# UniBwTAS/continuous_clustering

Measured on AMD Instinct MI355X. Metric: Mpoints/s clustered (64-beam streams), higher is better.
Workload: dtype f32

## Files before the change

continuous_clustering_amd/csrc/cc_k_assoc_global.h:

```cpp
#pragma once

constexpr int LINK_SLOTS_V1 = 8;

struct AssocCtx
{
    SP p;
    int R, NC, RC;
    float az_width, maxd2;
    int max_steps_in_row, max_steps_in_column, stop_enabled, stop_min_steps;
};

__device__ __forceinline__ int uf_find(int32_t* uf, int a)
{
    while (true)
    {
        const int pa = ld_agent(&uf[a]);
        if (pa == a)
            return a;
        const int gp = ld_agent(&uf[pa]);
        if (gp != pa)
            __hip_atomic_store(&uf[a], gp, __ATOMIC_RELAXED, __HIP_MEMORY_SCOPE_AGENT);
        a = pa;
    }
}
// ... 325 lines not shown
                    err = CC_ERR_CAPACITY;
                    err_a = n_unf + cnt;
                    break;
                }
                if (row < R)
                    p.root[lc * R + row] = active[k] ? rootc[k] : -1;
                if (is_new)
                {
                    const int cell = lc * R + row;
                    const int pos = n_unf + __popcll(mask & lanes_below());
                    const double fin = pcaz[k] + (double) mad[k];
                    tree_init(p, cell, fin);
                    p.ulist[pos] = cell;
                    p.t_pos[cell] = pos;
                    L = fin < L ? fin : L;
                }
                if (cnt > 0 && n_unf == 0)
                    M = gc;
                n_unf += cnt;
            }
            L = wave_min_f64(L);
            assoc_wave_sync();
#pragma unroll
            for (int k = 0; k < RPL; k++)
            {
                if (active[k] && parent[k] >= 0)
                {
                    const int r = rootc[k];
                    const long long rg = p.colg[r / R];
                    p.t_width[r] = (uint32_t) (gc - rg + 1);
                    const double cand = pcaz[k] + (double) mad[k];
                    atomicMax((unsigned long long*) &p.t_fin[r], (unsigned long long) __double_as_longlong(cand));
                    atomicAdd(&p.t_pts[r], 1u);
                }
            }
            assoc_wave_sync();
#pragma unroll
            for (int k = 0; k < RPL; k++)
            {
                const int row = k * 64 + lane;
                if (active[k] && parent[k] >= 0)
                {
                    const int rp = rootc[k];
                    for (int j = 0; j < nlinks[k]; j++)
                    {
                        const int rq = p.root[s_links[row][j]];
                        if (rq != rp && rq >= 0 && !p.t_finished[rp] && !p.t_finished[rq])
                        {
                            log_link(g, st, p.link_log, rp, rq);
                            uf_union(p.t_uf, rp, rq);
                        }
                    }
                }
            }
            assoc_wave_sync();
        }
        else
        {
            serial_cols++;
            if (lane == 0)
            {
                int nn = n_unf;
                double LL = L;
                long long MM = M;
                int e = 0;
                for (int row = 0; row < R; row++)
                {
                    const int ci = lc * R + row;
                    if (p.ignored[ci])
                    {
                        p.root[ci] = -1;
                        p.sc_parent[ci] = -2;
                        if (g.mirror_fields)
                            p.sc_visits[ci] = 0;
                        continue;
                    }
                    const float m = ccm::asinf_exact(cfg.max_distance / p.dist[ci]);
                    const double caz = cell_caz(cb, p.incaz[ci]);
                    int proot = -1, par = -1, nl = 0, vis = 0;
                    bool ov = false;
                    scan_point<true>(c, lc, gc, row, first_local, m, caz, proot, par, nullptr, nl, ov, LINK_SLOTS_V1, &vis, st, &g);
                    p.sc_parent[ci] = (int16_t) par;
                    if (g.mirror_fields)
                        p.sc_visits[ci] = sat_u16(vis);
                    if (proot == -1)
                    {
                        if (nn + 1 > g.tree_capacity)
                        {
                            e = CC_ERR_CAPACITY;
                            break;
                        }
                        proot = ci;
                        const double fin = caz + (double) m;
                        tree_init(p, ci, fin);
                        p.ulist[nn] = ci;
                        p.t_pos[ci] = nn;
                        if (nn == 0)
                            MM = gc;
                        nn++;
                        LL = fin < LL ? fin : LL;
                    }
                    p.root[ci] = proot;
                }
                s_bcast[0] = nn;
                s_bcast[1] = e;
                s_bd[0] = LL;
                s_bl[0] = MM;
            }
            assoc_wave_sync();
            n_unf = s_bcast[0];
            if (s_bcast[1])
            {
                err = s_bcast[1];
                err_a = n_unf;
            }
            L = s_bd[0];
            M = s_bl[0];
            assoc_wave_sync();
        }
        if (err)
            break;

        if (gc % nth != 0)
            continue;
        const double min_az = p.colminaz[lc];
        long long M_c;
        if (n_unf == 0)
            M_c = gc + 1;
        else if (min_az == last_min_az)
        {
            alias_rounds++;
            M_c = M;
        }
        else if (!(min_az >= L) && !((gc + 1 - M) >= NC))
            M_c = M;
        else
        {
            for (int i = lane; i < n_unf; i += 64)
            {
                p.agg_fin[i] = 0ull;
                p.agg_min[i] = 0x7fffffffffffffffll;
                p.agg_max[i] = 0;
                p.agg_pts[i] = 0;
                p.agg_first[i] = 0x7fffffff;
                p.agg_cid[i] = 0;
                p.agg_flag[i] = 0;
            }
            assoc_wave_sync();
            for (int i = lane; i < n_unf; i += 64)
            {
                const int t = p.ulist[i];
                const int rep = uf_find(p.t_uf, t);
                const int j = p.t_pos[rep];
                p.ucomp[i] = j;
                const long long tg = p.colg[t / R];
                atomicMax(&p.agg_fin[j], (unsigned long long) __double_as_longlong(ld_agent(&p.t_fin[t])));
                atomicMin(&p.agg_min[j], tg);
                atomicMax(&p.agg_max[j], tg + (long long) p.t_width[t]);
                atomicAdd(&p.agg_pts[j], ld_agent(&p.t_pts[t]));
                atomicMin(&p.agg_first[j], i);
            }
            assoc_wave_sync();
            int exceed_local = 0;
            for (int i = lane; i < n_unf; i += 64)
            {
                if (p.ucomp[i] == i)
                {
                    const double fin = __longlong_as_double((long long) ld_agent(&p.agg_fin[i]));
                    const bool unfinished = fin > min_az;
                    const bool exceeds = (ld_agent(&p.agg_max[i]) - ld_agent(&p.agg_min[i])) >= NC;
                    if (exceeds)
                        exceed_local++;
                    p.agg_flag[i] = (!unfinished || exceeds) ? 1 : 0;
                }
            }
            for (int o = 32; o > 0; o >>= 1)
                exceed_local += __shfl_xor(exceed_local, o);
            exceed += exceed_local;
            assoc_wave_sync();
            int last_first = -1;
            while (true)
            {
                int best = 0x7fffffff;
                for (int i = lane; i < n_unf; i += 64)
                    if (p.ucomp[i] == i && p.agg_flag[i] && ld_agent(&p.agg_pts[i]) > 5u)
                    {
                        const int fi = ld_agent(&p.agg_first[i]);
                        if (fi > last_first && fi < best)
                            best = fi;
                    }
                best = wave_min_i32(best);
                if (best == 0x7fffffff)
                    break;
                const int j = p.ucomp[best];
                const unsigned cid = (unsigned) cluster_counter;
                if (lane == 0)
                    p.agg_cid[j] = cid;
                emit(CC_EV_CLUSTER, ld_agent(&p.agg_min[j]), ld_agent(&p.agg_max[j]) - 1, cid, ld_agent(&p.agg_pts[j]), gc);
                cluster_counter++;
                clusters_finished++;
                last_first = best;
            }
            assoc_wave_sync();
            long long min_all = 0x7fffffffffffffffll, min_surv = 0x7fffffffffffffffll;
            double L_new = 1.7976931348623157e308;
            int out = 0;
            for (int base = 0; base < n_unf; base += 64)
            {
                const int i = base + lane;
                bool surv = false;
                int t = -1;
                if (i < n_unf)
                {
                    t = p.ulist[i];
                    const int j = p.ucomp[i];
                    const long long tg = p.colg[t / R];
                    min_all = tg < min_all ? tg : min_all;
                    if (p.agg_flag[j])
                    {
                        p.t_finished[t] = 1;
                        p.t_cid[t] = p.agg_cid[j];
                    }
                    else
                    {
                        surv = true;
                        min_surv = tg < min_surv ? tg : min_surv;
                        if (j == i)
                        {
                            const double fin = __longlong_as_double((long long) ld_agent(&p.agg_fin[i]));
                            L_new = fin < L_new ? fin : L_new;
                        }
                    }
                }
                const unsigned long long mask = __ballot(surv);
                if (surv)
                {
                    const int np = out + __popcll(mask & lanes_below());
                    p.ulist[np] = t;
                    p.t_pos[t] = np;
                }
                out += __popcll(mask);
            }
            min_all = wave_min_i64(min_all);
            min_surv = wave_min_i64(min_surv);
            L = wave_min_f64(L_new);
            M_c = min_all;
            M = min_surv;
            n_unf = out;
            assoc_wave_sync();
        }
        last_min_az = min_az;

        if (M_c < first_unpub)
        {
            err = CC_ERR_BOOKKEEPING;
            err_a = M_c;
            err_b = first_unpub;
            break;
        }
        const long long old_unpub = first_unpub, old_ring = ring_start;
        first_unpub = M_c;
        ring_start = first_unpub - NC > 0 ? first_unpub - NC : 0;
        emit(CC_EV_PUBLISH_COLUMNS, old_unpub, first_unpub - 1, 0, 0, gc);
        cells_published += (unsigned long long) (first_unpub - old_unpub) * (unsigned long long) R;
        (void) old_ring;
    }

    if (lane == 0)
    {
        st->first_unpublished = first_unpub;
        st->batch[slot].pub_end = first_unpub;
        st->ring_start = ring_start;
        st->cluster_counter = cluster_counter;
        st->n_unfinished = n_unf;
        st->min_required = M;
        st->finish_lower_bound = L;
        st->last_round_min_az = last_min_az;
        st->cells_published = cells_published;
        st->clusters_finished = clusters_finished;
        st->exceed_one_rotation = exceed;
        st->serial_columns = serial_cols;
        st->stamp_alias_rounds = alias_rounds;
        st->batch[slot].acp_next = col_end;
        if (err == 0)
            st->assoc_mode = (cfg.max_steps_in_row > WIN_COLS - 2 || n_unf * 2 > g.lds_tree_limit) ? 1 : 0;
        st->n_events = n_events < g.event_capacity ? n_events : g.event_capacity;
        if (g.record_events && n_events > g.event_capacity && err == 0)
        {
            err = CC_ERR_CAPACITY;
            err_a = n_events;
        }
        if (err)
            raise_error(st, err, err_a, err_b);
    }
}

template<int RPL>
__global__ __launch_bounds__(64) void k_associate(Geometry g, cc_config cfg, Planes P, StreamState* states, int first_stream, int slot)
{
    associate_stream<RPL>(g, cfg, P, states, first_stream + (int) blockIdx.x, slot);
}


template<int RPL, bool MIRROR>
__device__ __forceinline__ void scan_column_epilogue(const SP& p, const int R, const int lc, const int lane, const int (&parent)[RPL],
                                                     const int (&nlinks)[RPL], const double (&fin)[RPL], const unsigned long long (&packed)[RPL],
                                                     int reach)
{
    int t[RPL];
#pragma unroll
    for (int k = 0; k < RPL; k++)
    {
        const int row = k * 64 + lane;
        const bool same_col = parent[k] >= 0 && (parent[k] >> 8) == 0;
        t[k] = same_col ? (parent[k] & 0xff) : row;
    }
    for (int it = 0; it < 7; it++)
    {
        int nt[RPL];
        bool changed = false;
#pragma unroll
        for (int k = 0; k < RPL; k++)
        {
            const int src = t[k];
            const int lo = __shfl(t[0], src & 63);
            const int hi = RPL > 1 ? __shfl(t[RPL - 1], src & 63) : lo;
            nt[k] = src < 64 ? lo : hi;
            changed |= nt[k] != t[k];
        }
#pragma unroll
        for (int k = 0; k < RPL; k++)
            t[k] = nt[k];
        if (!__any(changed))
            break;
    }
    int cnt_new = 0, mine[RPL];
    int max_delta = 0;
    int flags = 0;
    int n_act = 0;
    double newfin = 1.7976931348623157e308;
#pragma unroll
    for (int k = 0; k < RPL; k++)
    {
        n_act |= __popcll(__ballot(parent[k] >= -1)) << (8 * k);
        const bool is_new = parent[k] == -1;
        const unsigned long long mask = __ballot(is_new);
        const int newidx = cnt_new + __popcll(mask & lanes_below());
        cnt_new += __popcll(mask);
        mine[k] = is_new ? newidx : (parent[k] >= 0 ? parent[k] : -1);
        if (is_new && fin[k] < newfin)
            newfin = fin[k];
        if (parent[k] >= 0)
        {
            int d = parent[k] >> 8;
            const int nl = nlinks[k] == 255 ? LINK_SLOTS : nlinks[k];
            for (int j = 0; j < nl; j++)
            {
                const int dj = (int) ((packed[k] >> (16 * j + 8)) & 0xff);
                d = dj > d ? dj : d;
            }
            max_delta = d > max_delta ? d : max_delta;
        }
        if (nlinks[k] == 255)
            flags |= 1;
        else if (nlinks[k] > 0)
            flags |= 2;
    }
#pragma unroll
    for (int k = 0; k < RPL; k++)
    {
        const int row = k * 64 + lane;
        const int src = t[k];
        const int lo = __shfl(mine[0], src & 63);
        const int hi = RPL > 1 ? __shfl(mine[RPL - 1], src & 63) : lo;
        const int term = parent[k] < -1 ? -1 : (src < 64 ? lo : hi);
        if (row < R)
            p.sc_term[lc * R + row] = (int16_t) term;
        const unsigned long long actm = __ballot(parent[k] >= -1);
        if (parent[k] >= -1)
        {
            const int j = (k > 0 ? (n_act & 0xff) : 0) + __popcll(actm & lanes_below());
            const unsigned nlc = nlinks[k] == 255 ? 7u : (unsigned) nlinks[k];
            p.pk_meta[lc * R + j] = ((unsigned) term & 0xffffu) | ((unsigned) row << 16) | (nlc << 23) | (parent[k] == -1 ? 1u << 26 : 0u);
            p.pk_fin[lc * R + j] = fin[k];
            if (nlinks[k] > 0)
                p.pk_lk[lc * R + j] = packed[k];
        }
        else if (row < R)
            p.root[lc * R + row] = -1;
    }
    max_delta = -wave_min_i32(-max_delta);
    if (MIRROR)
        reach = -wave_min_i32(-reach);
    flags = (__any(flags & 1) ? 1 : 0) | (__any(flags & 2) ? 2 : 0);
    if (cnt_new > 0)
        newfin = wave_min_f64(newfin);
    if (lane == 0)
    {
        p.col_newfin[lc] = newfin;
        p.col_info[lc] = cnt_new | (flags << 8) | (max_delta << 16) | ((MIRROR ? reach : 0) << 24);
        p.col_act[lc] = (uint16_t) n_act;
    }
}
```

continuous_clustering_amd/csrc/cc_k_scan.h:

```cpp
#pragma once

#ifndef CC_SCAN_BLOCKS
#define CC_SCAN_BLOCKS 256
#endif
constexpr int SCAN_BLOCKS = CC_SCAN_BLOCKS;

template<int RPL, bool MIRROR>
__device__ __forceinline__ void scan_body(const Geometry& g, const cc_config& cfg, const Planes& P, StreamState* states, int first_stream, int slot,
                                          const int bx, const int by, const int ny)
{
    const int s = first_stream + bx;
    const int lane = lane_id();
    const StreamState* st = &states[s];
    if (st->error != 0 || st->batch[slot].seg_begin < 0 || st->batch[slot].mode != 0)
        return;
    AssocCtx c;
    c.p = stream_ptrs(P, g, s);
    const SP& p = c.p;
    const int R = c.R = g.num_rows;
    c.NC = g.num_columns;
    const int RC = c.RC = g.ring_cols;
    c.az_width = g.az_width;
    c.maxd2 = g.max_distance_squared;
    c.max_steps_in_row = cfg.max_steps_in_row;
// ... 171 lines not shown
                }
                for (int down = 0; down < 2; down++)
                {
                    if (down == 1 && sb == 0)
                        continue;
                    int d = (down == 1 || sb == 0) ? 1 : 0;
                    int run[2];
#pragma unroll
                    for (int k = 0; k < 2; k++)
                    {
                        const int orow = down ? k * 64 + lane + d : k * 64 + lane - d;
                        run[k] = (live_i[k] && orow >= 0 && orow < R && d <= c.max_steps_in_column) ? 1 : 0;
                    }
                    while (__any((run[0] | run[1]) != 0))
                    {
                        const int src = (down ? lane + d : lane - d) & 63;
                        const float a0x = __shfl(cr[0].x, src), a0y = __shfl(cr[0].y, src), a0z = __shfl(cr[0].z, src), a0w = __shfl(cr[0].w, src);
                        const float a1x = __shfl(cr[1].x, src), a1y = __shfl(cr[1].y, src), a1z = __shfl(cr[1].z, src), a1w = __shfl(cr[1].w, src);
#pragma unroll
                        for (int k = 0; k < 2; k++)
                        {
                            const int orow = down ? k * 64 + lane + d : k * 64 + lane - d;
                            const int half = orow >> 6;
                            const bool h1 = half == 1;
                            const float ox = h1 ? a1x : a0x, oy = h1 ? a1y : a0y, oz = h1 ? a1z : a0z, ow = h1 ? a1w : a0w;
                            if (MIRROR)
                            {
                                visits[k] += run[k];
                                reachk[k] = run[k] ? sb : reachk[k];
                            }
                            const int cont = (run[k] && !(ccm::absf(ow - me[k].w) > mad[k])) ? 1 : 0;
                            const float dx = me[k].x - ox, dy = me[k].y - oy, dz = me[k].z - oz;
                            const int acc = (cont && ox == ox && dx * dx + dy * dy + dz * dz < c.maxd2) ? 1 : 0;
                            const int cand = (sb << 8) | (orow & 0xff);
                            parent[k] = (acc && !rooted[k]) ? cand : parent[k];
                            if (__any(acc && rooted[k]))
                            {
                                const int as_link = (acc && rooted[k] && nlinks[k] < LINK_SLOTS) ? 1 : 0;
                                overflow[k] |= (acc && rooted[k] && nlinks[k] >= LINK_SLOTS) ? 1 : 0;
                                packed[k] |= as_link ? (unsigned long long) cand << (16 * nlinks[k]) : 0ull;
                                nlinks[k] += as_link;
                            }
                            rooted[k] |= acc;
                            const int stop = (rooted[k] && c.stop_enabled && d >= c.stop_min_steps) ? 1 : 0;
                            const int nrow = down ? orow + 1 : orow - 1;
                            run[k] = (cont && !stop && nrow >= 0 && nrow < R && d + 1 <= c.max_steps_in_column) ? 1 : 0;
                        }
                        d++;
                    }
                }
#pragma unroll
                for (int k = 0; k < 2; k++)
                    if (rooted[k] && c.stop_enabled && sb >= c.stop_min_steps)
                        live_i[k] = 0;
                if (oc == bound)
                    break;
                oc = oc == 0 ? RC - 1 : oc - 1;
            }
#pragma unroll
            for (int k = 0; k < 2; k++)
            {
                const int row = k * 64 + lane;
                if (overflow[k])
                    nlinks[k] = 255;
                if (inrow[k])
                {
                    const int ci = lc * R + row;
                    p.sc_parent[ci] = (int16_t) parent[k];
                    p.sc_nlinks[ci] = (uint8_t) nlinks[k];
                    if (g.scan_stores_fin)
                        p.sc_fin[ci] = fin[k];
                    if (nlinks[k] > 0)
                        p.sc_links[ci] = packed[k];
                    if (MIRROR)
                        p.sc_visits[ci] = sat_u16(visits[k]);
                }
                if (MIRROR)
                    reach = reachk[k] > reach ? reachk[k] : reach;
            }
        }
        scan_column_epilogue<RPL, MIRROR>(p, R, lc, lane, parent, nlinks, fin, packed, reach);
    }
}

template<int RPL, bool MIRROR>
__global__ __launch_bounds__(64) void k_scan(Geometry g, cc_config cfg, Planes P, StreamState* states, int first_stream, int slot)
{
    scan_body<RPL, MIRROR>(g, cfg, P, states, first_stream, slot, (int) blockIdx.x, (int) blockIdx.y, (int) gridDim.y);
}

__global__ __launch_bounds__(256) void k_small_front(Geometry g, cc_config cfg, Planes P, StreamState* states, int stream, int slot,
                                                     const float* __restrict__ xyz, const uint8_t* __restrict__ inten, const double* __restrict__ poses,
                                                     long long n, int* remaining, double* __restrict__ ego)
{
    const int R = g.num_rows;
    StreamState* st = &states[stream];
#ifdef CC_SF_STATS
    unsigned long long sf_t[6];
    sf_t[0] = __builtin_amdgcn_s_memtime();
#define SF_MARK(i) sf_t[i] = __builtin_amdgcn_s_memtime();
#else
#define SF_MARK(i)
#endif
    if (threadIdx.x == 0)
    {
        st->cursor = 0;
        st->par_bad = 0x7fffffff;
        st->par_upto = -1;
        st->par_clear_done = -1;
        st->pre_seg_begin = 0;
        st->n_events = 0;
        st->n_links = 0;
        st->batch[slot].fused = 0;
        st->clear_allowed = st->ring_start;
        *remaining = 0;
    }
    for (long long f = threadIdx.x; f < n; f += 256)
        ego_record(states, stream, cfg, poses, n, n, 0, ego, 0, f);
    for (long long i = threadIdx.x; i < n * R; i += 256)
    {
        const PreppedPoint q = prep_point(xyz[i * 3 + 0], xyz[i * 3 + 1], xyz[i * 3 + 2], poses + (i / R) * 12, cfg.sensor_is_clockwise != 0, g.az_width);
        P.pp_cir[i] = q.cir;
        if (q.cir == PP_SKIP)
            continue;
        P.pp_x[i] = q.x;
        P.pp_y[i] = q.y;
        P.pp_z[i] = q.z;
        P.pp_dist[i] = q.dist;
        P.pp_incl[i] = q.incl;
        P.pp_incaz[i] = q.incaz;
    }
    if (threadIdx.x == 0)
    {
        long long* w = insert2_sync_words<1>(R);
        lds_st(w, 0ll);
        lds_st(w + 1, 0ll);
        lds_st(w + 2, -1ll);
    }
    __syncthreads();
    SF_MARK(1)
    if (threadIdx.x < 128)
        insert2_body<1, true, true>(g, cfg, P, states, stream, slot, inten, n, remaining, n, 0, 0);
    __syncthreads();
    SF_MARK(2)
    if (threadIdx.x < 64)
        seg_small_body(g, cfg, P, states, stream, slot, poses, n, 0, ego, n, 0);
    __syncthreads();
    SF_MARK(3)
    if (g.mirror_fields)
        scan_body<1, true>(g, cfg, P, states, stream, slot, 0, uniform_i32((int) (threadIdx.x >> 6)), 4);
    else
        scan_body<1, false>(g, cfg, P, states, stream, slot, 0, uniform_i32((int) (threadIdx.x >> 6)), 4);
#ifdef CC_SF_STATS
    __syncthreads();
    SF_MARK(4)
    if (threadIdx.x == 0)
    {
        for (int i = 0; i < 4; i++)
            st->dbg[i] += sf_t[i + 1] - sf_t[i];
        st->dbg[4] += 1;
    }
#endif
}

#ifndef CC_SCAN_TILE_CELLS
#define CC_SCAN_TILE_CELLS 256
#endif
constexpr int SCAN_TILE_CELLS = CC_SCAN_TILE_CELLS;

struct ScanCfg
{
    int R, RC, max_col_steps, stop_min;
    bool stop_enabled;
    float maxd2;
};

struct ScanPoint
{
    float4 me;
    float mad;
    int row, needed, bound;
    int sb, down, d, oc, orow;
    int rooted, parent, nlinks, overflow, visits, reach;
    unsigned long long packed;
    bool run;

    __device__ __forceinline__ void next_column(const ScanCfg& c)
    {
        if ((rooted && c.stop_enabled && sb >= c.stop_min) || oc == bound || sb + 1 > needed)
            run = false;
        else
        {
            sb++;
            oc = oc == 0 ? c.RC - 1 : oc - 1;
            down = 0;
            d = 0;
            orow = row;
        }
    }
    __device__ __forceinline__ void next_direction(const ScanCfg& c)
    {
        if (down == 0 && sb > 0)
        {
            down = 1;
            d = 1;
            orow = row + 1;
            if (!(orow < c.R && d <= c.max_col_steps))
                next_column(c);
        }
        else
            next_column(c);
    }
    __device__ __forceinline__ void start(const ScanCfg& c, const bool have, const int lc)
    {
        sb = 0, down = 0, d = 1, oc = lc, orow = row - 1;
        rooted = 0, parent = -1, nlinks = 0, overflow = 0, visits = 0, reach = 0;
        packed = 0;
        run = have;
        if (run && !(orow >= 0 && d <= c.max_col_steps))
            next_direction(c);
    }
    template<bool MIRROR>
    __device__ __forceinline__ void step(const ScanCfg& c, const SP& p)
    {
        const float4 o = p.sc_rec[oc * c.R + orow];
        const unsigned char oign = p.ignored[oc * c.R + orow];
        if (MIRROR)
        {
            visits++;
            reach = sb;
        }
        if (ccm::absf(o.w - me.w) > mad)
            next_direction(c);
        else
        {
            const float dx = me.x - o.x, dy = me.y - o.y, dz = me.z - o.z;
            if (!oign && dx * dx + dy * dy + dz * dz < c.maxd2)
            {
                const int cand = (sb << 8) | orow;
                if (!rooted)
                    parent = cand;
                else if (nlinks < LINK_SLOTS)
                {
                    packed |= (unsigned long long) cand << (16 * nlinks);
                    nlinks++;
                }
                else
                    overflow = 1;
                rooted = 1;
            }
            if (rooted && c.stop_enabled && d >= c.stop_min)
                next_direction(c);
            else
            {
                d++;
                orow = down ? orow + 1 : orow - 1;
                if (!(orow >= 0 && orow < c.R && d <= c.max_col_steps))
                    next_direction(c);
            }
        }
    }
};

constexpr int SL_CAP = 8192;
struct ScanLongRec
{
    int ci;
    int oc;
    short orow, sb, d, needed;
    short parent;
    unsigned char down, rooted, nlinks, flags;
    float mad;
    unsigned long long packed;
};
static_assert(sizeof(ScanLongRec) == 40, "long-scan record");

#ifndef CC_SCAN_CAP
#define CC_SCAN_CAP 6
#endif
constexpr int SCAN_CAP = CC_SCAN_CAP;

template<int RPL, bool MIRROR, bool SPLIT = false>
__global__ __launch_bounds__(64) void k_scan2(Geometry g, cc_config cfg, Planes P, StreamState* states, int first_stream, int slot)
{
    static_assert(!(SPLIT && MIRROR), "the long-scan list does not carry the mirror's visit counts");
    const int s = first_stream + blockIdx.x;
    const int lane = lane_id();
    const StreamState* st = &states[s];
    if (st->error != 0 || st->batch[slot].seg_begin < 0 || st->batch[slot].mode != 0)
        return;
    const SP p = stream_ptrs(P, g, s);
    const int R = g.num_rows, RC = g.ring_cols;
    ScanCfg sc;
    sc.R = R, sc.RC = RC;
    sc.maxd2 = g.max_distance_squared;
    sc.max_col_steps = cfg.max_steps_in_column;
    sc.stop_enabled = cfg.stop_after_association_enabled != 0;
    sc.stop_min = cfg.stop_after_association_min_steps;
    const int max_row_steps = cfg.max_steps_in_row;
    const int TC = SCAN_TILE_CELLS / (RPL * 64);
    __shared__ unsigned short s_list[SCAN_TILE_CELLS];
    __shared__ short s_parent[SCAN_TILE_CELLS];
    __shared__ unsigned char s_nlinks[SCAN_TILE_CELLS];
    __shared__ unsigned short s_visits[MIRROR ? SCAN_TILE_CELLS : 1];
    __shared__ unsigned char s_reach[MIRROR ? SCAN_TILE_CELLS : 1];
    __shared__ double s_fin[SCAN_TILE_CELLS];
    __shared__ unsigned long long s_links[SCAN_TILE_CELLS];
    int* const sl_ctl = P.sl_ctl + (size_t) s * 4;
    ScanLongRec* const sl_rec = (ScanLongRec*) P.sl_rec + (size_t) s * SL_CAP;
    const long long col_begin = st->batch[slot].acp_next, col_end = st->batch[slot].seg_end, first_column = st->first_column;
    const int first_lc = (int) (first_column % RC);
    const long long n_tiles = (col_end - col_begin + TC - 1) / TC;
    for (long long tile = blockIdx.y; tile < n_tiles; tile += gridDim.y)
    {
        const long long gc0 = col_begin + tile * TC;
        const int ncols = (int) (col_end - gc0 < TC ? col_end - gc0 : TC);
        const int lc0 = (int) (gc0 % RC);
        const long long rot0 = gc0 / g.num_columns;
        const int cir0 = (int) (gc0 - rot0 * g.num_columns);
        int n_act = 0;
        for (int j = 0; j < TC * RPL; j++)
        {
            const int tc = j / RPL, row = (j % RPL) * 64 + lane;
            const int tl = tc * RPL * 64 + row;
            bool act = false;
            if (tc < ncols && row < R)
            {
                int lc = lc0 + tc;
                lc = lc >= RC ? lc - RC : lc;
                act = p.ignored[lc * R + row] == 0;
            }
            s_parent[tl] = -2;
            s_nlinks[tl] = 0;
            s_fin[tl] = 0.;
            s_links[tl] = 0;
            if (MIRROR)
            {
                s_visits[tl] = 0;
                s_reach[tl] = 0;
            }
            const unsigned long long m = __ballot(act);
            if (act)
                s_list[n_act + __popcll(m & lanes_below())] = (unsigned short) tl;
            n_act += __popcll(m);
        }
        wave_lds_fence();
        unsigned deferred = 0;
        for (int base = 0; base < n_act; base += 64)
        {
            const bool have = base + lane < n_act;
            const int tl = have ? (int) s_list[base + lane] : 0;
            const int tc = tl / (RPL * 64), row = tl % (RPL * 64);
            const long long gc = gc0 + tc;
            int lc = lc0 + tc;
            lc = lc >= RC ? lc - RC : lc;
            const int ci = lc * R + row;
            ScanPoint q;
            q.me = make_float4(0.f, 0.f, 0.f, 0.f);
            q.mad = 0.f;
            q.row = row;
            double fin = 0.;
            q.needed = -1;
            if (have)
            {
                q.me = p.sc_rec[ci];
                q.mad = ccm::asinf_exact(cfg.max_distance / p.dist[ci]);
                fin = cell_caz(caz_base_of_rotation(rot0 + (cir0 + tc >= g.num_columns ? 1 : 0)), p.incaz[ci]) + (double) q.mad;
                q.needed = f2i_x86(__builtin_ceilf(q.mad / g.az_width));
                q.needed = q.needed < max_row_steps ? q.needed : max_row_steps;
            }
            q.bound = (gc - first_column) <= (long long) max_row_steps + 1 ? first_lc : -1;
            q.start(sc, have, lc);
            bool pending = false;
            if (SPLIT)
            {
                for (int it = 0; it < g.scan_cap && __any(q.run); it++)
                    if (q.run)
                        q.template step<false>(sc, p);
                const unsigned long long m = __ballot(q.run);
                if (m)
                {
                    int lbase = 0;
                    if (lane == (int) __ffsll((long long) m) - 1)
                        lbase = atomicAdd(&sl_ctl[0], (int) __popcll(m));
                    lbase = __shfl(lbase, (int) __ffsll((long long) m) - 1);
                    const int idx = lbase + (int) __popcll(m & lanes_below());
                    if (q.run && idx < g.sl_cap)
                    {
                        ScanLongRec r;
                        r.ci = ci, r.oc = q.oc;
                        r.orow = (short) q.orow, r.sb = (short) q.sb, r.d = (short) q.d, r.needed = (short) q.needed;
                        r.parent = (short) q.parent;
                        r.down = (unsigned char) q.down, r.rooted = (unsigned char) q.rooted, r.nlinks = (unsigned char) q.nlinks;
                        r.flags = (unsigned char) ((q.overflow ? 1 : 0) | (q.bound >= 0 ? 2 : 0));
                        r.mad = q.mad;
                        r.packed = q.packed;
                        sl_rec[idx] = r;
                        pending = true;
                        q.run = false;
                    }
                    while (__any(q.run))
                        if (q.run)
                            q.template step<false>(sc, p);
                }
                for (int t2 = 0; t2 < TC; t2++)
                    if (__any(pending && tc == t2))
                        deferred |= 1u << t2;
            }
            else
            {
                while (__any(q.run))
                    if (q.run)
                        q.template step<MIRROR>(sc, p);
            }
            if (have)
            {
                s_parent[tl] = (short) (pending ? -3 : q.parent);
                s_nlinks[tl] = (unsigned char) (q.overflow ? 255 : q.nlinks);
                s_fin[tl] = fin;
                s_links[tl] = q.packed;
                if (MIRROR)
                {
                    s_visits[tl] = sat_u16(q.visits);
                    s_reach[tl] = (unsigned char) q.reach;
                }
            }
        }
        wave_lds_fence();
        for (int tc = 0; tc < ncols; tc++)
        {
            int lc = lc0 + tc;
            lc = lc >= RC ? lc - RC : lc;
            int parent[RPL], nlinks[RPL];
            double fin[RPL];
            unsigned long long packed[RPL];
            int reach = 0;
            const bool later = SPLIT && ((deferred >> tc) & 1u) != 0;
#pragma unroll
            for (int k = 0; k < RPL; k++)
            {
                const int row = k * 64 + lane;
                const int tl = tc * RPL * 64 + row;
                parent[k] = s_parent[tl];
                nlinks[k] = s_nlinks[tl];
                fin[k] = s_fin[tl];
                packed[k] = s_links[tl];
                if (MIRROR)
                    reach = (int) s_reach[tl] > reach ? (int) s_reach[tl] : reach;
                if (row < R)
                {
                    const int ci = lc * R + row;
                    if (g.scan_stores_fin)
                        p.sc_fin[ci] = fin[k];
                    if (!(later && parent[k] == -3))
                    {
                        p.sc_parent[ci] = (int16_t) parent[k];
                        p.sc_nlinks[ci] = (uint8_t) nlinks[k];
                        if (nlinks[k] > 0)
                            p.sc_links[ci] = packed[k];
                    }
                    if (MIRROR)
                        p.sc_visits[ci] = s_visits[tl];
                }
            }
            if (later)
            {
                if (lane == 0)
                    p.sl_cols[atomicAdd(&sl_ctl[2], 1)] = lc;
            }
            else
                scan_column_epilogue<RPL, MIRROR>(p, R, lc, lane, parent, nlinks, fin, packed, reach);
        }
        wave_lds_fence();
    }
}

#ifndef CC_SCAN_LONG_BLOCKS
#define CC_SCAN_LONG_BLOCKS 16
#endif
constexpr int SCAN_LONG_BLOCKS = CC_SCAN_LONG_BLOCKS;
constexpr int SCAN_EPI_BLOCKS = 16;

template<int RPL>
__global__ __launch_bounds__(64) void k_scan2_long(Geometry g, cc_config cfg, Planes P, StreamState* states, int first_stream, int slot, int* __restrict__ stat)
{
    const int s = first_stream + blockIdx.x;
    int* const sl_ctl = P.sl_ctl + (size_t) s * 4;
    int n = sl_ctl[0];
    if (n <= 0)
        return;
    n = n < g.sl_cap ? n : g.sl_cap;
    const StreamState* st = &states[s];
    const int lane = lane_id();
    const SP p = stream_ptrs(P, g, s);
    const ScanLongRec* const sl_rec = (ScanLongRec*) P.sl_rec + (size_t) s * SL_CAP;
    const int R = g.num_rows, RC = g.ring_cols;
    ScanCfg sc;
    sc.R = R, sc.RC = RC;
    sc.maxd2 = g.max_distance_squared;
    sc.max_col_steps = cfg.max_steps_in_column;
    sc.stop_enabled = cfg.stop_after_association_enabled != 0;
    sc.stop_min = cfg.stop_after_association_min_steps;
    const int first_lc = (int) (st->first_column % RC);
    ScanPoint q;
    q.run = false;
    q.me = make_float4(0.f, 0.f, 0.f, 0.f);
    q.mad = 0.f, q.row = 0, q.needed = 0, q.bound = -1, q.sb = 0, q.down = 0, q.d = 0, q.oc = 0, q.orow = 0;
    q.rooted = 0, q.parent = -1, q.nlinks = 0, q.overflow = 0, q.visits = 0, q.reach = 0, q.packed = 0ull;
    int ci = 0;
    int nvis = 0;
    bool more = true;
    for (;;)
    {
        const unsigned long long idle = __ballot(!q.run);
        if (more && idle)
        {
            int lbase = 0;
            if (lane == (int) __ffsll((long long) idle) - 1)
                lbase = atomicAdd(&sl_ctl[1], (int) __popcll(idle));
            lbase = __shfl(lbase, (int) __ffsll((long long) idle) - 1);
            const int idx = lbase + (int) __popcll(idle & lanes_below());
            if (!q.run && idx < n)
            {
                const ScanLongRec r = sl_rec[idx];
                ci = r.ci;
                q.me = p.sc_rec[ci];
                q.mad = r.mad;
                q.row = ci % R;
                q.needed = r.needed;
                q.bound = (r.flags & 2) ? first_lc : -1;
                q.sb = r.sb, q.down = r.down, q.d = r.d, q.oc = r.oc, q.orow = r.orow;
                q.rooted = r.rooted, q.parent = r.parent, q.nlinks = r.nlinks, q.overflow = r.flags & 1;
                q.packed = r.packed;
                q.run = true;
            }
            more = lbase + (int) __popcll(idle) < n;
        }
        if (!__any(q.run))
            break;
        for (int it = 0; it < 8; it++)
            if (q.run)
            {
                q.template step<false>(sc, p);
                nvis++;
                if (!q.run)
                {
                    p.sc_parent[ci] = (int16_t) q.parent;
                    p.sc_nlinks[ci] = (uint8_t) (q.overflow ? 255 : q.nlinks);
                    if (q.nlinks > 0)
                        p.sc_links[ci] = q.packed;
                }
            }
    }
    if (stat)
    {
        for (int off = 32; off > 0; off >>= 1)
            nvis += __shfl_down(nvis, off, 64);
        if (lane == 0 && nvis > 0)
            atomicAdd(&stat[1], nvis);
    }
}

template<int RPL>
__global__ __launch_bounds__(64) void k_scan2_epi(Geometry g, cc_config cfg, Planes P, StreamState* states, int first_stream, int slot, int* __restrict__ stat)
{
    const int s = first_stream + blockIdx.x;
    int* const sl_ctl = P.sl_ctl + (size_t) s * 4;
    const int nd = sl_ctl[2];
    const int lane = lane_id();
    if (stat && blockIdx.y == 0 && lane == 0)
    {
        const StreamState* st = &states[s];
        if (st->error == 0 && st->batch[slot].seg_begin >= 0 && st->batch[slot].mode == 0)
        {
            atomicAdd(&stat[2], (int) (st->batch[slot].seg_end - st->batch[slot].acp_next));
        }
    }
    if (nd <= 0 && sl_ctl[0] <= 0)
        return;
    const SP p = stream_ptrs(P, g, s);
    const int R = g.num_rows;
    for (int i = blockIdx.y; i < nd; i += gridDim.y)
    {
        const int lc = p.sl_cols[i];
        const CazBase cb = caz_base_of_column(p.colg[lc], g.num_columns);
        int parent[RPL], nlinks[RPL];
        double fin[RPL];
        unsigned long long packed[RPL];
#pragma unroll
        for (int k = 0; k < RPL; k++)
        {
            const int row = k * 64 + lane;
            parent[k] = -2, nlinks[k] = 0, fin[k] = 0., packed[k] = 0ull;
            if (row < R)
            {
                const int ci = lc * R + row;
                parent[k] = p.sc_parent[ci];
                nlinks[k] = p.sc_nlinks[ci];
                fin[k] = cell_fin(cfg, p, ci, cb);
                if (nlinks[k] > 0)
                    packed[k] = p.sc_links[ci];
            }
        }
        scan_column_epilogue<RPL, false>(p, R, lc, lane, parent, nlinks, fin, packed, 0);
    }
    __threadfence();
    if (lane == 0 && atomicAdd(&sl_ctl[3], 1) == (int) gridDim.y - 1)
    {
        sl_ctl[0] = 0;
        sl_ctl[1] = 0;
        sl_ctl[2] = 0;
        sl_ctl[3] = 0;
    }
}
```

Before: 17510.

## Compact scan tile epilogue over active cells with wave-shuffle root resolution

When a 256-cell non-mirror tile has at most 128 active points, scan results are stored compactly by active index instead of by cell position. A new packed epilogue resolves parent chains by pointer jumping with wave shuffles, computes terminal ids, packed metadata and per-column summaries from the compact list, and writes ignored cells directly in the first pass. This avoids clearing the whole tile in LDS and the per-column loop over every cell. In exchange it adds shuffle iterations, LDS atomics and a second code path that aliases shared buffers.

```diff
diff --git a/continuous_clustering_amd/csrc/cc_k_assoc_global.h b/continuous_clustering_amd/csrc/cc_k_assoc_global.h
--- a/continuous_clustering_amd/csrc/cc_k_assoc_global.h
+++ b/continuous_clustering_amd/csrc/cc_k_assoc_global.h
@@ -751,3 +751,180 @@
         p.col_act[lc] = (uint16_t) n_act;
     }
 }
+
+__device__ __forceinline__ unsigned long long lanes_below_n(const int n)
+{
+    return n <= 0 ? 0ull : (n >= 64 ? ~0ull : (1ull << n) - 1ull);
+}
+
+constexpr int SCAN_LIST_SHIFT = 9;
+template<int TC>
+struct ScanTile
+{
+    const unsigned short* list;
+    const unsigned char* rowpos;
+    const short* parent;
+    const unsigned char* nlinks;
+    const double* fin;
+    const unsigned long long* links;
+    int* colsum;
+    unsigned ends;
+    unsigned act;
+    int lc0, ncols;
+    unsigned deferred;
+    __device__ __forceinline__ int begin(const int c) const { return c == 0 ? 0 : (int) ((ends >> (8 * (c - 1))) & 0xffu); }
+    __device__ __forceinline__ int end(const int c) const { return (int) ((ends >> (8 * c)) & 0xffu); }
+};
+
+template<int RPL, bool SPLIT, int TC>
+__device__ __forceinline__ void scan_tile_epilogue_packed(const SP& p, const bool stores_fin, const int R, const int RC, const int lane,
+                                                          const ScanTile<TC>& T)
+{
+    static_assert(TC * RPL == 4 && TC <= 4, "a tile of 256 cells");
+    constexpr int NS = 2;
+    const int n_pts = T.end(TC - 1);
+    const bool two = n_pts > 64;
+    int e[NS], parent[NS], t[NS];
+#pragma unroll
+    for (int k = 0; k < NS; k++)
+    {
+        const int pos = k * 64 + lane;
+        e[k] = 0, parent[k] = -2, t[k] = pos;
+        if ((k == 0 || two) && pos < n_pts)
+        {
+            e[k] = T.list[pos];
+            parent[k] = T.parent[pos];
+            const int tc = (e[k] & ((1 << SCAN_LIST_SHIFT) - 1)) / (RPL * 64);
+            const bool later = SPLIT && ((T.deferred >> tc) & 1u) != 0;
+            if (!later && parent[k] >= 0 && (parent[k] >> 8) == 0)
+                t[k] = T.rowpos[tc * RPL * 64 + (parent[k] & 0xff)];
+        }
+    }
+    for (int it = 0; it < 7; it++)
+    {
+        int nt[NS];
+        bool changed = false;
+#pragma unroll
+        for (int k = 0; k < NS; k++)
+        {
+            nt[k] = t[k];
+            if (k == 0 || two)
+            {
+                const int src = t[k];
+                const int lo = __shfl(t[0], src & 63);
+                const int hi = two ? __shfl(t[1], src & 63) : lo;
+                nt[k] = src < 64 ? lo : hi;
+                changed |= nt[k] != t[k];
+            }
+        }
+#pragma unroll
+        for (int k = 0; k < NS; k++)
+            t[k] = nt[k];
+        if (!__any(changed))
+            break;
+    }
+    const unsigned long long new0 = __ballot(parent[0] == -1), new1 = two ? __ballot(parent[1] == -1) : 0ull;
+    unsigned new_before = 0;
+#pragma unroll
+    for (int c = 1; c < TC; c++)
+        new_before |= (unsigned) (__popcll(new0 & lanes_below_n(T.begin(c))) + __popcll(new1 & lanes_below_n(T.begin(c) - 64))) << (8 * c);
+    int mine[NS];
+#pragma unroll
+    for (int k = 0; k < NS; k++)
+    {
+        const int tc = (e[k] & ((1 << SCAN_LIST_SHIFT) - 1)) / (RPL * 64);
+        const int idx = (k == 0 ? 0 : (int) __popcll(new0)) + (int) __popcll((k == 0 ? new0 : new1) & lanes_below()) - (int) ((new_before >> (8 * tc)) & 0xffu);
+        mine[k] = parent[k] == -1 ? idx : (parent[k] >= 0 ? parent[k] : -1);
+    }
+    int term[NS];
+#pragma unroll
+    for (int k = 0; k < NS; k++)
+    {
+        term[k] = -1;
+        if (k == 0 || two)
+        {
+            const int src = t[k];
+            const int lo = __shfl(mine[0], src & 63);
+            const int hi = two ? __shfl(mine[1], src & 63) : lo;
+            term[k] = src < 64 ? lo : hi;
+        }
+    }
+#pragma unroll
+    for (int k = 0; k < NS; k++)
+    {
+        const int pos = k * 64 + lane;
+        if (!((k == 0 || two) && pos < n_pts))
+            continue;
+        const int tl = e[k] & ((1 << SCAN_LIST_SHIFT) - 1);
+        const int tc = tl / (RPL * 64), row = tl % (RPL * 64);
+        int lc = T.lc0 + tc;
+        lc = lc >= RC ? lc - RC : lc;
+        const int ci = lc * R + row, pkj = lc * R + (e[k] >> SCAN_LIST_SHIFT);
+        const bool later = SPLIT && ((T.deferred >> tc) & 1u) != 0;
+        const int nlinks = T.nlinks[pos];
+        const double fin = T.fin[pos];
+        const unsigned long long packed = T.links[pos];
+        if (stores_fin)
+            p.sc_fin[ci] = fin;
+        if (!(later && parent[k] == -3))
+        {
+            p.sc_parent[ci] = (int16_t) parent[k];
+            p.sc_nlinks[ci] = (uint8_t) nlinks;
+            if (nlinks > 0)
+                p.sc_links[ci] = packed;
+        }
+        if (later)
+            continue;
+        p.sc_term[ci] = (int16_t) term[k];
+        const unsigned nlc = nlinks == 255 ? 7u : (unsigned) nlinks;
+        p.pk_meta[pkj] = ((unsigned) term[k] & 0xffffu) | ((unsigned) row << 16) | (nlc << 23) | (parent[k] == -1 ? 1u << 26 : 0u);
+        p.pk_fin[pkj] = fin;
+        if (nlinks > 0)
+            p.pk_lk[pkj] = packed;
+        if (parent[k] >= 0)
+        {
+            int d = parent[k] >> 8;
+            const int nl = nlinks == 255 ? LINK_SLOTS : nlinks;
+            for (int j = 0; j < nl; j++)
+            {
+                const int dj = (int) ((packed >> (16 * j + 8)) & 0xff);
+                d = dj > d ? dj : d;
+            }
+            if (d > 0)
+                atomicMax(&T.colsum[tc], d);
+        }
+        if (nlinks > 0)
+            atomicOr(&T.colsum[TC + tc], nlinks == 255 ? 1 : 2);
+    }
+#pragma unroll
+    for (int c = 0; c < TC; c++)
+    {
+        if (c >= T.ncols || (SPLIT && ((T.deferred >> c) & 1u) != 0))
+            continue;
+        int lc = T.lc0 + c;
+        lc = lc >= RC ? lc - RC : lc;
+        const int b = T.begin(c), en = T.end(c);
+        const int cnt_new = (int) (__popcll(new0 & lanes_below_n(en) & ~lanes_below_n(b)) + __popcll(new1 & lanes_below_n(en - 64) & ~lanes_below_n(b - 64)));
+        double newfin = 1.7976931348623157e308;
+        if (cnt_new > 0)
+        {
+#pragma unroll
+            for (int k = 0; k < NS; k++)
+            {
+                const int pos = k * 64 + lane;
+                if ((k == 0 || two) && parent[k] == -1 && pos >= b && pos < en)
+                {
+                    const double fin = T.fin[pos];
+                    newfin = fin < newfin ? fin : newfin;
+                }
+            }
+            newfin = wave_min_f64(newfin);
+        }
+        if (lane == 0)
+        {
+            p.col_newfin[lc] = newfin;
+            p.col_info[lc] = cnt_new | (T.colsum[TC + c] << 8) | (T.colsum[c] << 16);
+            p.col_act[lc] = (uint16_t) ((T.act >> ((32 / TC) * c)) & ((1u << (32 / TC)) - 1u));
+        }
+    }
+}
diff --git a/continuous_clustering_amd/csrc/cc_k_scan.h b/continuous_clustering_amd/csrc/cc_k_scan.h
--- a/continuous_clustering_amd/csrc/cc_k_scan.h
+++ b/continuous_clustering_amd/csrc/cc_k_scan.h
@@ -501,6 +501,9 @@
     __shared__ unsigned char s_reach[MIRROR ? SCAN_TILE_CELLS : 1];
     __shared__ double s_fin[SCAN_TILE_CELLS];
     __shared__ unsigned long long s_links[SCAN_TILE_CELLS];
+    constexpr bool PACKED = !MIRROR && SCAN_TILE_CELLS == 256;
+    unsigned char* const s_rowpos = reinterpret_cast<unsigned char*>(&s_parent[SCAN_TILE_CELLS / 2]);
+    int* const s_colsum = reinterpret_cast<int*>(&s_fin[SCAN_TILE_CELLS / 2]);
     int* const sl_ctl = P.sl_ctl + (size_t) s * 4;
     ScanLongRec* const sl_rec = (ScanLongRec*) P.sl_rec + (size_t) s * SL_CAP;
     const long long col_begin = st->batch[slot].acp_next, col_end = st->batch[slot].seg_end, first_column = st->first_column;
@@ -513,38 +516,73 @@
         const int lc0 = (int) (gc0 % RC);
         const long long rot0 = gc0 / g.num_columns;
         const int cir0 = (int) (gc0 - rot0 * g.num_columns);
+        ScanTile<TC> T;
+        T.list = s_list, T.rowpos = s_rowpos, T.parent = s_parent, T.nlinks = s_nlinks, T.fin = s_fin, T.links = s_links, T.colsum = s_colsum;
+        T.lc0 = lc0, T.ncols = ncols, T.ends = 0, T.act = 0;
+        int col_base = 0;
         int n_act = 0;
+#pragma unroll
         for (int j = 0; j < TC * RPL; j++)
         {
             const int tc = j / RPL, row = (j % RPL) * 64 + lane;
             const int tl = tc * RPL * 64 + row;
+            if (j % RPL == 0)
+                col_base = n_act;
             bool act = false;
             if (tc < ncols && row < R)
             {
                 int lc = lc0 + tc;
                 lc = lc >= RC ? lc - RC : lc;
-                act = p.ignored[lc * R + row] == 0;
-            }
-            s_parent[tl] = -2;
-            s_nlinks[tl] = 0;
-            s_fin[tl] = 0.;
-            s_links[tl] = 0;
-            if (MIRROR)
-            {
-                s_visits[tl] = 0;
-                s_reach[tl] = 0;
+                const int ci = lc * R + row;
+                act = p.ignored[ci] == 0;
+                if (PACKED && !act)
+                {
+                    p.sc_parent[ci] = (int16_t) -2;
+                    p.sc_nlinks[ci] = (uint8_t) 0;
+                    p.sc_term[ci] = (int16_t) -1;
+                    p.root[ci] = -1;
+                    if (g.scan_stores_fin)
+                        p.sc_fin[ci] = 0.;
+                }
             }
             const unsigned long long m = __ballot(act);
             if (act)
-                s_list[n_act + __popcll(m & lanes_below())] = (unsigned short) tl;
-            n_act += __popcll(m);
-        }
+            {
+                const int pos = n_act + (int) __popcll(m & lanes_below());
+                s_list[pos] = (unsigned short) (tl | ((pos - col_base) << SCAN_LIST_SHIFT));
+                if (PACKED)
+                    s_rowpos[tl] = (unsigned char) pos;
+            }
+            n_act += (int) __popcll(m);
+            T.act |= (unsigned) __popcll(m) << ((32 / TC) * tc + 8 * (j % RPL));
+            if (j % RPL == RPL - 1)
+                T.ends |= (unsigned) (n_act & 0xff) << (8 * tc);
+        }
+        const bool pk = PACKED && n_act <= 128;
+        if (pk)
+        {
+            if (lane < 2 * TC)
+                s_colsum[lane] = 0;
+        }
+        else
+            for (int tl = lane; tl < SCAN_TILE_CELLS; tl += 64)
+            {
+                s_parent[tl] = -2;
+                s_nlinks[tl] = 0;
+                s_fin[tl] = 0.;
+                s_links[tl] = 0;
+                if (MIRROR)
+                {
+                    s_visits[tl] = 0;
+                    s_reach[tl] = 0;
+                }
+            }
         wave_lds_fence();
         unsigned deferred = 0;
         for (int base = 0; base < n_act; base += 64)
         {
             const bool have = base + lane < n_act;
-            const int tl = have ? (int) s_list[base + lane] : 0;
+            const int tl = have ? (int) s_list[base + lane] & ((1 << SCAN_LIST_SHIFT) - 1) : 0;
             const int tc = tl / (RPL * 64), row = tl % (RPL * 64);
             const long long gc = gc0 + tc;
             int lc = lc0 + tc;
@@ -610,10 +648,11 @@
             }
             if (have)
             {
-                s_parent[tl] = (short) (pending ? -3 : q.parent);
-                s_nlinks[tl] = (unsigned char) (q.overflow ? 255 : q.nlinks);
-                s_fin[tl] = fin;
-                s_links[tl] = q.packed;
+                const int at = pk ? base + lane : tl;
+                s_parent[at] = (short) (pending ? -3 : q.parent);
+                s_nlinks[at] = (unsigned char) (q.overflow ? 255 : q.nlinks);
+                s_fin[at] = fin;
+                s_links[at] = q.packed;
                 if (MIRROR)
                 {
                     s_visits[tl] = sat_u16(q.visits);
@@ -622,50 +661,65 @@
             }
         }
         wave_lds_fence();
-        for (int tc = 0; tc < ncols; tc++)
-        {
-            int lc = lc0 + tc;
-            lc = lc >= RC ? lc - RC : lc;
-            int parent[RPL], nlinks[RPL];
-            double fin[RPL];
-            unsigned long long packed[RPL];
-            int reach = 0;
-            const bool later = SPLIT && ((deferred >> tc) & 1u) != 0;
-#pragma unroll
-            for (int k = 0; k < RPL; k++)
-            {
-                const int row = k * 64 + lane;
-                const int tl = tc * RPL * 64 + row;
-                parent[k] = s_parent[tl];
-                nlinks[k] = s_nlinks[tl];
-                fin[k] = s_fin[tl];
-                packed[k] = s_links[tl];
-                if (MIRROR)
-                    reach = (int) s_reach[tl] > reach ? (int) s_reach[tl] : reach;
-                if (row < R)
-                {
-                    const int ci = lc * R + row;
-                    if (g.scan_stores_fin)
-                        p.sc_fin[ci] = fin[k];
-                    if (!(later && parent[k] == -3))
+        if (pk)
+        {
+            T.deferred = deferred;
+            if constexpr (PACKED)
+                scan_tile_epilogue_packed<RPL, SPLIT, TC>(p, g.scan_stores_fin != 0, R, RC, lane, T);
+            if (SPLIT && deferred != 0 && lane == 0)
+                for (int tc = 0; tc < ncols; tc++)
+                    if ((deferred >> tc) & 1u)
                     {
-                        p.sc_parent[ci] = (int16_t) parent[k];
-                        p.sc_nlinks[ci] = (uint8_t) nlinks[k];
-                        if (nlinks[k] > 0)
-                            p.sc_links[ci] = packed[k];
+                        int lc = lc0 + tc;
+                        lc = lc >= RC ? lc - RC : lc;
+                        p.sl_cols[atomicAdd(&sl_ctl[2], 1)] = lc;
                     }
+        }
+        else
+            for (int tc = 0; tc < ncols; tc++)
+            {
+                int lc = lc0 + tc;
+                lc = lc >= RC ? lc - RC : lc;
+                int parent[RPL], nlinks[RPL];
+                double fin[RPL];
+                unsigned long long packed[RPL];
+                int reach = 0;
+                const bool later = SPLIT && ((deferred >> tc) & 1u) != 0;
+#pragma unroll
+                for (int k = 0; k < RPL; k++)
+                {
+                    const int row = k * 64 + lane;
+                    const int tl = tc * RPL * 64 + row;
+                    parent[k] = s_parent[tl];
+                    nlinks[k] = s_nlinks[tl];
+                    fin[k] = s_fin[tl];
+                    packed[k] = s_links[tl];
                     if (MIRROR)
-                        p.sc_visits[ci] = s_visits[tl];
-                }
-            }
-            if (later)
-            {
-                if (lane == 0)
-                    p.sl_cols[atomicAdd(&sl_ctl[2], 1)] = lc;
-            }
-            else
-                scan_column_epilogue<RPL, MIRROR>(p, R, lc, lane, parent, nlinks, fin, packed, reach);
-        }
+                        reach = (int) s_reach[tl] > reach ? (int) s_reach[tl] : reach;
+                    if (row < R)
+                    {
+                        const int ci = lc * R + row;
+                        if (g.scan_stores_fin)
+                            p.sc_fin[ci] = fin[k];
+                        if (!(later && parent[k] == -3))
+                        {
+                            p.sc_parent[ci] = (int16_t) parent[k];
+                            p.sc_nlinks[ci] = (uint8_t) nlinks[k];
+                            if (nlinks[k] > 0)
+                                p.sc_links[ci] = packed[k];
+                        }
+                        if (MIRROR)
+                            p.sc_visits[ci] = s_visits[tl];
+                    }
+                }
+                if (later)
+                {
+                    if (lane == 0)
+                        p.sl_cols[atomicAdd(&sl_ctl[2], 1)] = lc;
+                }
+                else
+                    scan_column_epilogue<RPL, MIRROR>(p, R, lc, lane, parent, nlinks, fin, packed, reach);
+            }
         wave_lds_fence();
     }
 }
```

Result: slower. 17210 (-1.7%).

## Write fin and link outputs directly from scan lanes instead of staging in LDS

Applied to the files above, without the earlier changes.

Drops the per-cell fin (double) and links (u64) shared-memory staging arrays from the scan tile. Each lane now writes pk_fin, pk_lk, sc_links and sc_fin straight to global memory. It computes the per-cell max delta into a small byte array, and reduces each column's minimum new-cluster fin with wave reductions. The goal is to cut LDS footprint and traffic, which may improve occupancy, and to remove redundant per-column work in the epilogue. The cost is scattered global stores from the compacted active list, plus extra per-column ballot and wave-min loops. The packed index also relies on a column-start prefix being correct.

```diff
diff --git a/continuous_clustering_amd/csrc/cc_k_assoc_global.h b/continuous_clustering_amd/csrc/cc_k_assoc_global.h
--- a/continuous_clustering_amd/csrc/cc_k_assoc_global.h
+++ b/continuous_clustering_amd/csrc/cc_k_assoc_global.h
@@ -651,10 +651,10 @@
 }
 
 
-template<int RPL, bool MIRROR>
+template<int RPL, bool MIRROR, bool PRE = false>
 __device__ __forceinline__ void scan_column_epilogue(const SP& p, const int R, const int lc, const int lane, const int (&parent)[RPL],
                                                      const int (&nlinks)[RPL], const double (&fin)[RPL], const unsigned long long (&packed)[RPL],
-                                                     int reach)
+                                                     int reach, const int* const maxd = nullptr, const double newfin_pre = 0.)
 {
     int t[RPL];
 #pragma unroll
@@ -687,7 +687,7 @@
     int max_delta = 0;
     int flags = 0;
     int n_act = 0;
-    double newfin = 1.7976931348623157e308;
+    double newfin = PRE ? newfin_pre : 1.7976931348623157e308;
 #pragma unroll
     for (int k = 0; k < RPL; k++)
     {
@@ -697,9 +697,14 @@
         const int newidx = cnt_new + __popcll(mask & lanes_below());
         cnt_new += __popcll(mask);
         mine[k] = is_new ? newidx : (parent[k] >= 0 ? parent[k] : -1);
-        if (is_new && fin[k] < newfin)
+        if (!PRE && is_new && fin[k] < newfin)
             newfin = fin[k];
-        if (parent[k] >= 0)
+        if (PRE)
+        {
+            if (parent[k] >= 0)
+                max_delta = maxd[k] > max_delta ? maxd[k] : max_delta;
+        }
+        else if (parent[k] >= 0)
         {
             int d = parent[k] >> 8;
             const int nl = nlinks[k] == 255 ? LINK_SLOTS : nlinks[k];
@@ -731,9 +736,12 @@
             const int j = (k > 0 ? (n_act & 0xff) : 0) + __popcll(actm & lanes_below());
             const unsigned nlc = nlinks[k] == 255 ? 7u : (unsigned) nlinks[k];
             p.pk_meta[lc * R + j] = ((unsigned) term & 0xffffu) | ((unsigned) row << 16) | (nlc << 23) | (parent[k] == -1 ? 1u << 26 : 0u);
-            p.pk_fin[lc * R + j] = fin[k];
-            if (nlinks[k] > 0)
-                p.pk_lk[lc * R + j] = packed[k];
+            if (!PRE)
+            {
+                p.pk_fin[lc * R + j] = fin[k];
+                if (nlinks[k] > 0)
+                    p.pk_lk[lc * R + j] = packed[k];
+            }
         }
         else if (row < R)
             p.root[lc * R + row] = -1;
@@ -742,7 +750,7 @@
     if (MIRROR)
         reach = -wave_min_i32(-reach);
     flags = (__any(flags & 1) ? 1 : 0) | (__any(flags & 2) ? 2 : 0);
-    if (cnt_new > 0)
+    if (!PRE && cnt_new > 0)
         newfin = wave_min_f64(newfin);
     if (lane == 0)
     {
@@ -751,3 +759,12 @@
         p.col_act[lc] = (uint16_t) n_act;
     }
 }
+
+template<int RPL, bool MIRROR>
+__device__ __forceinline__ void scan_column_epilogue_packed(const SP& p, const int R, const int lc, const int lane, const int (&parent)[RPL],
+                                                            const int (&nlinks)[RPL], const int (&maxd)[RPL], const double newfin, int reach)
+{
+    const double no_fin[RPL] = {};
+    const unsigned long long no_links[RPL] = {};
+    scan_column_epilogue<RPL, MIRROR, true>(p, R, lc, lane, parent, nlinks, no_fin, no_links, reach, maxd, newfin);
+}
diff --git a/continuous_clustering_amd/csrc/cc_k_scan.h b/continuous_clustering_amd/csrc/cc_k_scan.h
--- a/continuous_clustering_amd/csrc/cc_k_scan.h
+++ b/continuous_clustering_amd/csrc/cc_k_scan.h
@@ -497,10 +497,9 @@
     __shared__ unsigned short s_list[SCAN_TILE_CELLS];
     __shared__ short s_parent[SCAN_TILE_CELLS];
     __shared__ unsigned char s_nlinks[SCAN_TILE_CELLS];
+    __shared__ unsigned char s_maxd[SCAN_TILE_CELLS];
     __shared__ unsigned short s_visits[MIRROR ? SCAN_TILE_CELLS : 1];
     __shared__ unsigned char s_reach[MIRROR ? SCAN_TILE_CELLS : 1];
-    __shared__ double s_fin[SCAN_TILE_CELLS];
-    __shared__ unsigned long long s_links[SCAN_TILE_CELLS];
     int* const sl_ctl = P.sl_ctl + (size_t) s * 4;
     ScanLongRec* const sl_rec = (ScanLongRec*) P.sl_rec + (size_t) s * SL_CAP;
     const long long col_begin = st->batch[slot].acp_next, col_end = st->batch[slot].seg_end, first_column = st->first_column;
@@ -514,10 +513,14 @@
         const long long rot0 = gc0 / g.num_columns;
         const int cir0 = (int) (gc0 - rot0 * g.num_columns);
         int n_act = 0;
+        int col_start[TC];
+#pragma unroll
         for (int j = 0; j < TC * RPL; j++)
         {
             const int tc = j / RPL, row = (j % RPL) * 64 + lane;
             const int tl = tc * RPL * 64 + row;
+            if (j % RPL == 0)
+                col_start[tc] = n_act;
             bool act = false;
             if (tc < ncols && row < R)
             {
@@ -527,8 +530,6 @@
             }
             s_parent[tl] = -2;
             s_nlinks[tl] = 0;
-            s_fin[tl] = 0.;
-            s_links[tl] = 0;
             if (MIRROR)
             {
                 s_visits[tl] = 0;
@@ -541,6 +542,7 @@
         }
         wave_lds_fence();
         unsigned deferred = 0;
+        double col_newfin = 1.7976931348623157e308;
         for (int base = 0; base < n_act; base += 64)
         {
             const bool have = base + lane < n_act;
@@ -612,23 +614,58 @@
             {
                 s_parent[tl] = (short) (pending ? -3 : q.parent);
                 s_nlinks[tl] = (unsigned char) (q.overflow ? 255 : q.nlinks);
-                s_fin[tl] = fin;
-                s_links[tl] = q.packed;
                 if (MIRROR)
                 {
                     s_visits[tl] = sat_u16(q.visits);
                     s_reach[tl] = (unsigned char) q.reach;
                 }
-            }
+                if (g.scan_stores_fin)
+                    p.sc_fin[ci] = fin;
+            }
+            const bool done = have && !pending;
+            if (done)
+            {
+                int cs = col_start[0];
+#pragma unroll
+                for (int t2 = 1; t2 < TC; t2++)
+                    cs = tc >= t2 ? col_start[t2] : cs;
+                const int j = base + lane - cs;
+                p.pk_fin[lc * R + j] = fin;
+                if (q.nlinks > 0)
+                {
+                    p.pk_lk[lc * R + j] = q.packed;
+                    p.sc_links[ci] = q.packed;
+                }
+                if (q.parent >= 0)
+                {
+                    int dmax = q.parent >> 8;
+                    const int nl = q.overflow ? LINK_SLOTS : q.nlinks;
+#pragma unroll
+                    for (int l = 0; l < LINK_SLOTS; l++)
+                        if (l < nl)
+                        {
+                            const int dl = (int) ((q.packed >> (16 * l + 8)) & 0xff);
+                            dmax = dl > dmax ? dl : dmax;
+                        }
+                    s_maxd[tl] = (unsigned char) dmax;
+                }
+            }
+            const bool is_new = done && q.parent == -1;
+#pragma unroll
+            for (int t2 = 0; t2 < TC; t2++)
+                if (__any(is_new && tc == t2))
+                {
+                    const double m = wave_min_f64(is_new && tc == t2 && fin < 1.7976931348623157e308 ? fin : 1.7976931348623157e308);
+                    if (lane == t2 && m < col_newfin)
+                        col_newfin = m;
+                }
         }
         wave_lds_fence();
         for (int tc = 0; tc < ncols; tc++)
         {
             int lc = lc0 + tc;
             lc = lc >= RC ? lc - RC : lc;
-            int parent[RPL], nlinks[RPL];
-            double fin[RPL];
-            unsigned long long packed[RPL];
+            int parent[RPL], nlinks[RPL], maxd[RPL];
             int reach = 0;
             const bool later = SPLIT && ((deferred >> tc) & 1u) != 0;
 #pragma unroll
@@ -638,21 +675,18 @@
                 const int tl = tc * RPL * 64 + row;
                 parent[k] = s_parent[tl];
                 nlinks[k] = s_nlinks[tl];
-                fin[k] = s_fin[tl];
-                packed[k] = s_links[tl];
+                maxd[k] = s_maxd[tl];
                 if (MIRROR)
                     reach = (int) s_reach[tl] > reach ? (int) s_reach[tl] : reach;
                 if (row < R)
                 {
                     const int ci = lc * R + row;
-                    if (g.scan_stores_fin)
-                        p.sc_fin[ci] = fin[k];
+                    if (g.scan_stores_fin && parent[k] == -2)
+                        p.sc_fin[ci] = 0.;
                     if (!(later && parent[k] == -3))
                     {
                         p.sc_parent[ci] = (int16_t) parent[k];
                         p.sc_nlinks[ci] = (uint8_t) nlinks[k];
-                        if (nlinks[k] > 0)
-                            p.sc_links[ci] = packed[k];
                     }
                     if (MIRROR)
                         p.sc_visits[ci] = s_visits[tl];
@@ -664,7 +698,7 @@
                     p.sl_cols[atomicAdd(&sl_ctl[2], 1)] = lc;
             }
             else
-                scan_column_epilogue<RPL, MIRROR>(p, R, lc, lane, parent, nlinks, fin, packed, reach);
+                scan_column_epilogue_packed<RPL, MIRROR>(p, R, lc, lane, parent, nlinks, maxd, __shfl(col_newfin, tc), reach);
         }
         wave_lds_fence();
     }
```

After: 18350 before, 18060 after. 1.5% lower.
